# coganlab/cross_patient_speech_decoding

Hardware: AMD Instinct MI355X
Metric: ECoG trials/sec seq2seq-RNN training (higher is better)
Workload: dtype bf16x3; 1 GPU; configs[3] per-GPU shard: 8-patient MCCA-aligned input (d = 30), enc 2x bi-GRU H=512, dec 1x GRU, T=200 (T'=20), F=100, full-batch step of 2048 trials per GPU (8 patients x 2048 trials over 8 GPUs), dropout 0.3, teacher forcing 0.5, clip 0.5, AdamW; trials_per_gpu=2048, global_batch=2048, parallelism=dp1, collective=none (single process)

## Files before the change

cross_patient_speech_decoding_amd/nn_models/functional.py:

```python
import ctypes as C
from typing import NamedTuple

import torch

from .._dev import need_gpu as _need_gpu, ptr as _ptr, ptr_array as _ptr_array, stream as _stream, workspace as _ws
from .. import _switches
from .._lib import TnProblem, call, lib, rowmap

_f32 = torch.float32

GEMM_PRECISIONS = {'fp32': 0, 'bf16x3': 1}


def set_gemm_precision(name):
    if name not in GEMM_PRECISIONS:
        raise ValueError(f"gemm precision must be one of {sorted(GEMM_PRECISIONS)}")
    call('xps_set_gemm_precision', GEMM_PRECISIONS[name])


def get_gemm_precision():
    mode = lib().xps_get_gemm_precision()
    return {v: k for k, v in GEMM_PRECISIONS.items()}[mode]


# ... 340 lines not shown
        return dgi, dghn, dh0
    call('xps_gru_seq_bwd_f32', _ptr(dy), _ptr(dhn), _ptr(y_ext), _ptr(saved), _ptr_array(w_hh), _ptr_array(w_t), _ptr(dgi),
         _ptr(dghn), _ptr(dh0), T, B, H, ndir, _ptr(ws), nbytes, _stream())
    return dgi, dghn, dh0


def _recurrent_grad_problems(dgi, dghn, y_ext, w_hh_params, b_hh_params, T, B, H, ndir, fmt=0, y_fmt=0):
    dev = y_ext.device
    ldy = ndir * H
    probs, rets = [], []
    for d in range(ndir):
        dw, db, acc_w, rw, rb = _grad_targets(w_hh_params[d], (3 * H, H), b_hh_params[d], (3 * H,), dev)
        first_slot = 0 if d == 0 else 2
        hprev = y_ext.view(-1)[first_slot * B * ldy + d * H:]
        probs.append(tn_problem(dgi[d], hprev, dw, 2 * H, H, T * B, ra=rowmap(3 * H, fmt=fmt), rb=rowmap(ldy, fmt=y_fmt), rc=rowmap(H),
                                colsum_out=db, accumulate=acc_w))
        probs.append(tn_problem(dghn[d], hprev, dw[2 * H:], H, H, T * B, ra=rowmap(H, fmt=fmt), rb=rowmap(ldy, fmt=y_fmt), rc=rowmap(H),
                                colsum_out=db[2 * H:], accumulate=acc_w))
        rets.append((rw, rb))
    return probs, rets


class GRURecurFn(torch.autograd.Function):

    @staticmethod
    def forward(ctx, gi, h0, ndir, *wb):
        _need_gpu(gi, h0, *wb)
        w_hh = [w.contiguous() for w in wb[:ndir]]
        b_hh = [b.contiguous() for b in wb[ndir:]]
        gi = gi.contiguous()
        _, T, B, H3 = gi.shape
        H = H3 // 3
        h0c = None if h0 is None else h0.contiguous()
        save = any(ctx.needs_input_grad)
        y_ext, saved = _gru_forward(gi, w_hh, b_hh, h0c, T, B, H, ndir, save)
        if save:
            ctx.save_for_backward(y_ext, saved, *w_hh)
            ctx.form = saved.launch_form
        ctx.params = wb
        ctx.dims = (T, B, H, ndir)
        ctx.has_h0 = h0 is not None
        return y_ext

    @staticmethod
    def backward(ctx, dy_ext):
        y_ext, saved, *w_hh = ctx.saved_tensors
        T, B, H, ndir = ctx.dims
        need_dh0 = ctx.has_h0 and ctx.needs_input_grad[1]
        dgi, dghn, dh0 = _gru_backward(dy_ext[1:T + 1], None, y_ext, saved, w_hh, T, B, H, ndir, need_dh0, form=ctx.form)
        if need_dh0:
            dh0[0] += dy_ext[0, :, :H]
            if ndir == 2:
                dh0[1] += dy_ext[T + 1, :, H:]
        probs, rets = _recurrent_grad_problems(dgi, dghn, y_ext, ctx.params[:ndir], ctx.params[ndir:], T, B, H, ndir)
        gemm_tn_grouped(probs, y_ext.device)
        return (dgi, dh0, None, *[r[0] for r in rets], *[r[1] for r in rets])


HN_NONE, HN_STACK, HN_SUM = 0, 1, 2


FMT_X_SPLIT4, FMT_Y_SPLIT4 = 1, 2


def split4_mode():
    return lib().xps_get_gemm_precision() == 1 and bool(_switches.get('XPS_SPLIT4'))


def layer_output_split4_ok(T, B, H, ndir, drop_p):
    return bool(drop_p and drop_p > 0.0 and split4_mode() and H > 256 and (ndir * H) % 4 == 0
                and not fused_dropout_supported(T, B, H, ndir))


def _presplit_weights_ok(rows, In, H3):
    return (split4_mode() and In % 4 == 0 and rows >= 4096 and In * H3 >= _switches.get('XPS_SPLIT4_WEIGHTS_MIN')
            and bool(_switches.get('XPS_SPLIT4_WEIGHTS')))


def skinny_dx_wanted(rows, In, K):
    return (bool(_switches.get('XPS_SKINNY_DX')) and split4_mode() and In % 4 == 0 and In < 256 and rows % 256 == 0
            and rows >= 96 * 256 and K % 32 == 0 and K >= 512 and bool(_switches.get('XPS_GEMM_DMA')))


def split4_pad(w, ldo):
    w = w.contiguous()
    out = torch.empty(w.shape[0], ldo, dtype=_f32, device=w.device)
    call('xps_split4_pad_f32', _ptr(w), w.shape[1], w.shape[0], w.shape[1], _ptr(out), ldo, _stream())
    return out


def split4(x, drop_p=0.0, seed=0):
    out = torch.empty_like(x)
    call('xps_split4_f32', _ptr(x), _ptr(out), x.numel(), float(drop_p), int(seed), _stream())
    return out


class GruPlan(NamedTuple):
    cluster_on: bool
    precision: int
    drop_fused: bool
    x_fmt: int
    w_fmt: int
    y_out_split: bool
    fwd_images: bool
    fwd_ysplit: bool
    want_dropped: bool
    bwd_split4: int
    y_fmt: int
    skinny_dx: bool


def gru_layer_plan(T, B, In, H, ndir, drop_p, fmt):
    has_drop = bool(drop_p and drop_p > 0.0)
    drop_fused = bool(has_drop and fused_dropout_supported(T, B, H, ndir))
    y_out_split = bool(fmt & FMT_Y_SPLIT4)
    if y_out_split and (not has_drop or drop_fused):
        raise ValueError('FMT_Y_SPLIT4: only with a separate dropout pass (see layer_output_split4_ok)')
    w_fmt = 1 if _presplit_weights_ok(T * B, In, 3 * H) else 0
    split4 = bool(split4_wanted(T, B, H, ndir))
    hprev = bool(hprev_split_wanted(T, B, H, ndir, split4))
    fwd_images = bool(fwd_images_wanted(T, B, H, ndir, hprev))
    return GruPlan(cluster_on=lib().xps_get_gru_cluster_mode() != 0, precision=lib().xps_get_gemm_precision(), drop_fused=drop_fused,
                   x_fmt=1 if (fmt & FMT_X_SPLIT4) else 0, w_fmt=w_fmt, y_out_split=y_out_split, fwd_images=fwd_images,
                   fwd_ysplit=bool(fwd_ysplit_wanted(T, B, H, ndir, hprev)), want_dropped=fwd_images and y_out_split,
                   bwd_split4=int(split4), y_fmt=int(hprev),
                   skinny_dx=bool(split4 and not w_fmt and skinny_dx_wanted(T * B, In, 3 * H)))


class GRULayerFmtFn(torch.autograd.Function):

    @staticmethod
    def forward(ctx, x, ndir, hn_mode, drop_p, fmt, *wb):
        ctx.set_materialize_grads(False)
        _need_gpu(x, *wb)
        x = x.contiguous()
        T, B, In = x.shape
        w_ih = [wb[4 * d + 0].contiguous() for d in range(ndir)]
        w_hh = [wb[4 * d + 1].contiguous() for d in range(ndir)]
        b_ih = [wb[4 * d + 2].contiguous() for d in range(ndir)]
        b_hh = [wb[4 * d + 3].contiguous() for d in range(ndir)]
        H = w_hh[0].shape[1]
        plan = ctx.plan = gru_layer_plan(T, B, In, H, ndir, drop_p, fmt)
        gi = torch.empty(ndir, T, B, 3 * H, dtype=_f32, device=x.device)
        if plan.w_fmt:
            w_ih = [split4(w) for w in w_ih]
        ra, rb, rc = rowmap(In, fmt=plan.x_fmt), rowmap(In, fmt=plan.w_fmt), rowmap(3 * H)
        call('xps_gemm_nt_multi_f32', _ptr(x), C.byref(ra), _ptr_array(w_ih), C.byref(rb), _ptr_array([gi[d] for d in range(ndir)]),
             C.byref(rc), _ptr_array(b_ih), ndir, T * B, 3 * H, In, _stream())
        save = any(ctx.needs_input_grad)
        drop = None
        y_drop = None
        if drop_p and drop_p > 0.0:
            drop = (float(drop_p), next_dropout_seed())
        ctx.drop = drop
        y_split = None
        if (save and (plan.fwd_images or plan.fwd_ysplit)) or plan.want_dropped:
            y_ext, saved, y_split, y_drop = _gru_forward_images(gi, w_hh, b_hh, T, B, H, ndir, save, plan.want_dropped, drop)
        elif plan.drop_fused:
            y_ext, saved, y_drop = _gru_forward(gi, w_hh, b_hh, None, T, B, H, ndir, save, drop)
        else:
            y_ext, saved = _gru_forward(gi, w_hh, b_hh, None, T, B, H, ndir, save)
        if save:
            ctx.save_for_backward(x, y_ext, saved, *w_ih, *w_hh, *([y_split] if y_split is not None else []))
        ctx.params = wb
        ctx.dims = (T, B, H, ndir, In, hn_mode)
        y = y_ext[1:T + 1]
        if y_drop is not None:
            y = y_drop
        elif drop is not None:
            out = torch.empty(T, B, ndir * H, dtype=_f32, device=x.device)
            if plan.y_out_split:
                call('xps_split4_f32', _ptr(y), _ptr(out), out.numel(), drop[0], drop[1], _stream())
            else:
                call('xps_dropout_f32', _ptr(y), _ptr(out), None, out.numel(), drop[0], drop[1], _stream())
            y = out
        if hn_mode == HN_NONE:
            hn = None
        elif hn_mode == HN_SUM:
            hn = y_ext[T, :, :H] + y_ext[1, :, H:] if ndir == 2 else y_ext[T, :, :H].clone()
        else:
            hn = torch.stack([y_ext[T, :, :H]] + ([y_ext[1, :, H:]] if ndir == 2 else []), dim=0)
        return y, hn

    @staticmethod
    def backward(ctx, dy, dhn):
        T, B, H, ndir, In, hn_mode = ctx.dims
        if dhn is not None and hn_mode == HN_SUM:
            dhn = dhn.unsqueeze(0).expand(ndir, B, H).contiguous()
        plan = ctx.plan
        if lib().xps_get_gemm_precision() != plan.precision:
            names = {v: k for k, v in GEMM_PRECISIONS.items()}
            raise RuntimeError(f'GRU backward: the forward chose its operand formats in {names[plan.precision]} mode but the backward '
                               f'runs in {names[lib().xps_get_gemm_precision()]} mode: the product precision (set_gemm_precision / '
                               'XPS_GEMM_PRECISION) must not change between a forward and its backward')
        x, y_ext, saved, *w = ctx.saved_tensors
        y_split = w.pop() if (plan.fwd_images or plan.fwd_ysplit) else None
        w_ih, w_hh = w[:ndir], w[ndir:]
        fmt, y_fmt, x_fmt, w_fmt = plan.bwd_split4, plan.y_fmt, plan.x_fmt, plan.w_fmt
        wb = ctx.params
        if ctx.drop is not None and dy is not None and not plan.drop_fused:
            dyc = dy.contiguous()
            dyd = torch.empty_like(dyc)
            call('xps_dropout_f32', _ptr(dyc), _ptr(dyd), None, dyc.numel(), ctx.drop[0], ctx.drop[1], _stream())
            dy = dyd
        dgi, dghn, _ = _gru_backward(dy, dhn, y_ext, saved, w_hh, T, B, H, ndir, False, ctx.drop if plan.drop_fused else None,
                                     split4=bool(fmt), form=(plan.cluster_on, B, H))
        dev = x.device
        have_img = y_split is not None
        y_src = (y_split if have_img else torch.empty_like(y_ext)) if y_fmt else y_ext
        probs, rets_hh = _recurrent_grad_problems(dgi, dghn, y_src, [wb[4 * d + 1] for d in range(ndir)],
                                                  [wb[4 * d + 3] for d in range(ndir)], T, B, H, ndir, fmt, y_fmt)
        rets_ih = []
        for d in range(ndir):
            dw, db, acc_w, rw, rb = _grad_targets(wb[4 * d + 0], (3 * H, In), wb[4 * d + 2], (3 * H,), dev)
            probs.append(tn_problem(dgi[d], x, dw, 3 * H, In, T * B, ra=rowmap(3 * H, fmt=fmt), rb=rowmap(In, fmt=x_fmt),
                                    colsum_out=db, accumulate=acc_w))
            rets_ih.append((rw, rb))
        direct = all(r[0] is None and r[1] is None for r in rets_ih + rets_hh)
        def launch_group(st):
            if y_fmt and not have_img:
                call('xps_split4_f32', _ptr(y_ext), _ptr(y_src), y_ext.numel(), 0.0, 0, _stream() if st is None else st)
            return gemm_tn_grouped(probs, dev, st)
        _launch_weight_grads(launch_group, dev, (dgi, dghn, x, y_ext, y_src), direct)
        dx = None
        if ctx.needs_input_grad[0]:
            dx = torch.empty(T, B, In, dtype=_f32, device=dev)
            if plan.skinny_dx:
                w_ih = [split4_pad(w, 256) for w in w_ih]
                w_fmt, ldw = 1, 256
            else:
                ldw = In
            if ndir == 2:
                ra, rb, rc = rowmap(3 * H, fmt=fmt), rowmap(ldw, fmt=w_fmt), rowmap(In)
                call('xps_gemm_nn2_f32', _ptr(dgi[0]), _ptr(w_ih[0]), 3 * H, _ptr(dgi[1]), _ptr(w_ih[1]), 3 * H,
                     C.byref(ra), C.byref(rb), _ptr(dx), C.byref(rc), T * B, In, 0, _stream())
            else:
                gemm_nn(dgi[0], w_ih[0], dx, T * B, In, 3 * H, ra=rowmap(3 * H, fmt=fmt), rb=rowmap(ldw, fmt=w_fmt))
        grads = []
        for d in range(ndir):
            grads += [rets_ih[d][0], rets_hh[d][0], rets_ih[d][1], rets_hh[d][1]]
        return (dx, None, None, None, None, *grads)


class GRULayerDropFn(torch.autograd.Function):

    @staticmethod
    def forward(ctx, x, ndir, hn_mode, drop_p, *wb):
        return GRULayerFmtFn.forward(ctx, x, ndir, hn_mode, drop_p, 0, *wb)

    @staticmethod
    def backward(ctx, dy, dhn):
        g = GRULayerFmtFn.backward(ctx, dy, dhn)
        return g[:4] + g[5:]


class GRULayerFn(torch.autograd.Function):

    @staticmethod
    def forward(ctx, x, ndir, hn_mode, *wb):
        return GRULayerDropFn.forward(ctx, x, ndir, hn_mode, 0.0, *wb)

    @staticmethod
    def backward(ctx, dy, dhn):
        g = GRULayerDropFn.backward(ctx, dy, dhn)
        return g[:3] + g[4:]


POST_SYNCBN_HOOKS = []
def _dp_world(group):
    import torch.distributed as dist
    if group is not None and dist.is_available() and dist.is_initialized():
        return dist.get_world_size(group)
    return 1


def _dp_enabled(group):
    return _dp_world(group) > 1


def _dist_sum_(t, group):
    if _dp_enabled(group):
        import torch.distributed as dist
        dist.all_reduce(t, op=dist.ReduceOp.SUM, group=group)
        return True
    return False


def _global_rows(rows, group, device, global_trials, Tp):
    if global_trials is not None:
        return float(global_trials) * Tp
    cnt = torch.tensor([float(rows)], dtype=torch.float64, device=device)
    _dist_sum_(cnt, group)
    return float(cnt.item())


class TemporalConvFn(torch.autograd.Function):

    @staticmethod
    def forward(ctx, x, conv_w, conv_b, gamma, beta, running_mean, running_var, stride, training,
                relu, drop_mask, drop_scale, momentum, eps, group, global_trials=None, num_batches_tracked=None):
        _need_gpu(x, conv_w)
        x = x.contiguous()
        B, T, Cin = x.shape
        F, _, k = conv_w.shape
        Tp = (T - k) // stride + 1
        if Tp < 1:
            raise ValueError('TemporalConv: sequence shorter than the kernel')
        w2 = conv_w.permute(0, 2, 1).contiguous().view(F, k * Cin)
        rows = Tp * B
        y = torch.empty(Tp, B, F, dtype=_f32, device=x.device)
        ra = rowmap(stride * Cin, rpg=Tp, gs=T * Cin)
        rc = rowmap(B * F, rpg=Tp, gs=F)
        gemm_nt(x, w2, y, rows, F, k * Cin, bias=conv_b, ra=ra, rc=rc)
        out = torch.empty_like(y)
        if training:
            stats = torch.empty(2 * F, dtype=_f32, device=x.device)
            nbytes = lib().xps_colsum_f32_workspace(rows, F)
            ws = _ws(nbytes, x.device)
            call('xps_colsum_f32', _ptr(y), F, rows, F, _ptr(stats), None, 0, _ptr(ws), nbytes, _stream())
            count = float(rows)
# ... 729 lines not shown
```

include/xps.h:

```cpp
#ifndef XPS_H
#define XPS_H

#include <stddef.h>
#include <stdint.h>

#ifdef __cplusplus
extern "C" {
#endif

#define XPS_OK 0
#define XPS_E_INVALID (-1)
#define XPS_E_HIP (-2)
#define XPS_E_WORKSPACE (-3)

typedef struct xps_rowmap {
    int64_t gs;
    int64_t ld;
    int32_t rpg;
    int32_t fmt;
} xps_rowmap;
#define XPS_FMT_F32 0
#define XPS_FMT_SPLIT4 1

const char* xps_last_error(void);
int xps_abi_version(void);
int xps_stream_create_low_priority(void** stream);
int xps_stream_destroy(void* stream);
int xps_set_switch(const char* name, long long value);
int xps_get_switch(const char* name, long long* value);
int xps_list_switches(char* buf, size_t n);
int xps_set_gemm_precision(int mode);
int xps_get_gemm_precision(void);
int xps_set_gemm_big_tiles(int on);
int xps_get_gemm_big_tiles(void);


int xps_gemm_nt_f32(const float* A, const xps_rowmap* ra, const float* B, const xps_rowmap* rb,
                    float* C, const xps_rowmap* rc, const float* bias,
                    int M, int N, int K, int accumulate, void* stream);
int xps_gemm_nn_f32(const float* A, const xps_rowmap* ra, const float* B, const xps_rowmap* rb,
                    float* C, const xps_rowmap* rc,
                    int M, int N, int K, int accumulate, void* stream);
int xps_gemm_nt_multi_f32(const float* A, const xps_rowmap* ra, const float* const* B, const xps_rowmap* rb,
                          float* const* C, const xps_rowmap* rc, const float* const* bias, int nprob,
                          int M, int N, int K, void* stream);
int xps_gemm_nn2_f32(const float* A1, const float* B1, int K1, const float* A2, const float* B2, int K2,
                     const xps_rowmap* ra, const xps_rowmap* rb, float* C, const xps_rowmap* rc,
                     int M, int N, int accumulate, void* stream);
size_t xps_gemm_tn_f32_workspace(int M, int N, int K);
int xps_gemm_tn_f32(const float* A, const xps_rowmap* ra, const float* B, const xps_rowmap* rb,
                    float* C, const xps_rowmap* rc,
                    int M, int N, int K, int accumulate,
                    void* workspace, size_t workspace_bytes, void* stream);

typedef struct xps_tn_problem {
    const float* A; const float* B; float* C; float* colsum_a;
    xps_rowmap ra, rb, rc;
    int32_t M, N, K, accumulate;
} xps_tn_problem;
size_t xps_gemm_tn_grouped_f32_workspace(const xps_tn_problem* probs, int n);
int xps_gemm_tn_grouped_f32(const xps_tn_problem* probs, int n, void* workspace, size_t workspace_bytes,
                            void* stream);

#define XPS_GEMM_FORM_NT 0
#define XPS_GEMM_FORM_NN 1
#define XPS_GEMM_FORM_NN2 2
#define XPS_GEMM_FORM_NT_MULTI 3
#define XPS_GEMM_ROUTE_REFUSED 0
#define XPS_GEMM_ROUTE_NONE 1
#define XPS_GEMM_ROUTE_SMALL_M 2
#define XPS_GEMM_ROUTE_SKINNY 3
#define XPS_GEMM_ROUTE_BIG 8
#define XPS_GEMM_ROUTE_BIG_DEEP 12
#define XPS_GEMM_ROUTE_BIG_DMA 13
#define XPS_GEMM_ROUTE_TILE 16
#define XPS_GEMM_ROUTE_TILE_128 1
#define XPS_GEMM_ROUTE_TILE_EDGE 2
#define XPS_GEMM_ROUTE_TILE_BF 4
#define XPS_GEMM_ROUTE_TILE_PRE 8
#define XPS_GEMM_ROUTE_PROJ_WS 32
int xps_gemm_route(int form, const float* A, const xps_rowmap* ra, const void* B, const xps_rowmap* rb, const float* A2,
                   const float* B2, const xps_rowmap* rc, int M, int N, int K, int K2, int nprob, int* lead_rows,
                   int* tail_route);
#define XPS_GEMM_TN_CLASS_128 0
#define XPS_GEMM_TN_CLASS_BIG 1
#define XPS_GEMM_TN_CLASS_BIG_DMA 2
#define XPS_GEMM_ROUTE_TN_EDGE 1
#define XPS_GEMM_ROUTE_TN_BF 2
#define XPS_GEMM_ROUTE_TN_PRE 4
#define XPS_GEMM_ROUTE_TN_DEEP 8
#define XPS_GEMM_ROUTE_TN_UNIFORM 16
#define XPS_GEMM_ROUTE_TN_FLAT 32
int xps_gemm_tn_grouped_route(const xps_tn_problem* probs, int n, int* cls, int* splits, int* kchunk);

size_t xps_colsum_f32_workspace(int rows, int cols);
int xps_colsum_f32(const float* X, int64_t ldx, int rows, int cols, float* out, float* out_sq,
                   int accumulate, void* workspace, size_t workspace_bytes, void* stream);

size_t xps_gru_seq_fwd_f32_workspace(int T, int B, int H, int ndir);
long long xps_gru_seq_status_offset(int T, int B, int H, int ndir);
int xps_gru_set_status_word(unsigned* device_word);
int xps_set_gru_bptt_grid(int two_dimensional);
int xps_get_gru_bptt_grid(void);
int xps_set_gru_cluster_mode(int mode);
int xps_get_gru_cluster_mode(void);
int xps_gru_seq_fwd_f32(const float* gi, const float* const* w_hh, const float* const* b_hh,
                        const float* h0, float* y_ext, float* saved,
                        int T, int B, int H, int ndir, void* workspace, size_t workspace_bytes, void* stream);

size_t xps_gru_seq_bwd_f32_workspace(int T, int B, int H, int ndir);
int xps_gru_seq_bwd_f32(const float* dy, const float* dhn, const float* y_ext, const float* saved,
                        const float* const* w_hh, const float* const* w_hh_t, float* dgi, float* dghn, float* dh0,
                        int T, int B, int H, int ndir, void* workspace, size_t workspace_bytes, void* stream);
#define XPS_GRU_MAX_H_TILE 624
#define XPS_GRU_MAX_H_STEP 1264
#define XPS_GRU_ROUTE_REFUSED 0
#define XPS_GRU_ROUTE_CLUSTER 1
#define XPS_GRU_ROUTE_RESIDENT 2
#define XPS_GRU_ROUTE_GENERIC_VEC 3
#define XPS_GRU_ROUTE_GENERIC_SCALAR 4
#define XPS_GRU_ROUTE_STEP 8
#define XPS_GRU_ROUTE_STEP_VECA 1
#define XPS_GRU_ROUTE_STEP_VECB 2
int xps_gru_seq_route(int T, int B, int H, int ndir, int weights_aligned16, int backward);
int xps_gru_seq_fused_dropout_supported(int T, int B, int H, int ndir);
int xps_gru_seq_fwd_drop_f32(const float* gi, const float* const* w_hh, const float* const* b_hh,
                             const float* h0, float* y_ext, float* saved,
                             int T, int B, int H, int ndir, float* y_drop, float drop_p, uint64_t drop_seed,
                             void* workspace, size_t workspace_bytes, void* stream);
int xps_gru_seq_bwd_drop_f32(const float* dy, const float* dhn, const float* y_ext, const float* saved,
                             const float* const* w_hh, const float* const* w_hh_t, float* dgi, float* dghn, float* dh0,
                             int T, int B, int H, int ndir, float drop_p, uint64_t drop_seed,
                             void* workspace, size_t workspace_bytes, void* stream);
int xps_gru_seq_fwd_images_supported(int T, int B, int H, int ndir);
int xps_gru_seq_fwd_image_exchange_supported(int T, int B, int H, int ndir);
int xps_gru_seq_fwd_images_f32(const float* gi, const float* const* w_hh, const float* const* b_hh,
                               const float* h0, float* y_ext, float* saved, int T, int B, int H, int ndir,
                               float* y_split, float* y_drop_split, float drop_p, uint64_t drop_seed,
                               void* workspace, size_t workspace_bytes, void* stream);
int xps_gru_seq_bwd_split4_supported(int T, int B, int H, int ndir);
int xps_gru_seq_bwd_split4_f32(const float* dy, const float* dhn, const float* y_ext, const float* saved,
                               const float* const* w_hh, const float* const* w_hh_t, float* dgi, float* dghn, float* dh0,
                               int T, int B, int H, int ndir, float drop_p, uint64_t drop_seed,
                               void* workspace, size_t workspace_bytes, void* stream);

int xps_transpose_f32(const float* src, float* dst, int rows, int cols, void* stream);
int xps_transpose_batched_f32(const float* const* src, float* const* dst, int n, int rows, int cols, void* stream);

int xps_bn_centered_sumsq_f32(const float* y, int rows, int F, const float* stats, double count, float* out_sq,
                              void* workspace, size_t workspace_bytes, void* stream);
int xps_bn_finalize_f32(const float* stats, double count, float* mean, float* rstd,
                        float* running_mean, float* running_var, int64_t* num_batches_tracked,
                        float momentum, float eps, int F, void* stream);
int xps_bn_apply_f32(const float* y, const float* mean, const float* rstd,
                     const float* gamma, const float* beta, const float* drop_mask, float drop_scale,
                     float* out, int64_t rows, int F, int relu, void* stream);
int xps_bn_finalize_apply_f32(const float* y, const float* stats, double count, const float* gamma, const float* beta,
                              float* mean, float* rstd, float* running_mean, float* running_var,
                              int64_t* num_batches_tracked, float momentum, float eps, const float* drop_mask,
                              float drop_scale, float* out, int64_t rows, int F, int relu, void* stream);
int xps_bn_apply_eval_f32(const float* y, const float* running_mean, const float* running_var, float eps,
                          const float* gamma, const float* beta, float* out,
                          int64_t rows, int F, int relu, void* stream);
size_t xps_bn_bwd_workspace(int64_t rows, int F);
int xps_bn_bwd_reduce_f32(const float* dout, const float* out, const float* y, const float* mean,
                          const float* rstd, const float* drop_mask, float drop_scale, int relu,
                          float* sums, float* dbeta_acc, float* dgamma_acc, int64_t rows, int F,
                          void* workspace, size_t workspace_bytes, void* stream);
int xps_bn_bwd_apply_f32(const float* dout, const float* out, const float* y, const float* mean,
                         const float* rstd, const float* gamma, const float* drop_mask,
                         float drop_scale, int relu, const float* sums, double count,
                         float* dy, int64_t rows, int F, void* stream);

int xps_decoder_supported(int H, int C, int L);
int xps_decoder_fwd_f32(const float* table, const float* w_hh, const float* b_hh, const float* h0,
                        const float* w_fc, const float* b_fc, const int64_t* teacher, const int32_t* flags,
// ... 277 lines not shown
```

Measured before the change: 321,100 trials/s.

## Add dedicated skinny input-gradient kernels for narrow-input GRU layers

```diff
diff --git a/cross_patient_speech_decoding_amd/csrc/xps_gru_inputgrad.hip b/cross_patient_speech_decoding_amd/csrc/xps_gru_inputgrad.hip
--- /dev/null
+++ b/cross_patient_speech_decoding_amd/csrc/xps_gru_inputgrad.hip
@@ -0,0 +1,462 @@
+#include "xps_common.h"
+#include "xps_gemm_tile.h"
+#include "xps_gemm_dma.h"
+using namespace xps_tile;
+namespace {
+
+constexpr int IG_SLABS = 256;
+constexpr int IG_MAX_RG = 5;
+constexpr int IG_D = 4;
+constexpr int IG_B_IMG = 32 * 512;
+constexpr int ig_stage_bytes(int rg) { return rg * 32 * 128 + IG_B_IMG; }
+
+struct DxArgs {
+    const float* dgi[2];
+    const float* w[2];
+    float* dx;
+    int rows, In, H3, ndir;
+};
+
+inline int dx_row_groups(long long rows) {
+    long long rg = (rows + 32LL * IG_SLABS - 1) / (32LL * IG_SLABS);
+    return rg < 1 ? 1 : rg > IG_MAX_RG ? IG_MAX_RG : (int)rg;
+}
+
+template <int RG, bool PRE>
+__global__ __launch_bounds__(512, 2) void gru_dx_slab_kernel(const DxArgs a) {
+    extern __shared__ __attribute__((aligned(16))) unsigned char smem[];
+    constexpr int R = 32 * RG, A_IMG = R * 128, STAGE = A_IMG + IG_B_IMG;
+    constexpr int NP = RG + 4;
+    constexpr int NG = 2 * RG;
+    const int tid = threadIdx.x, lane = tid & 63;
+    const int wave8 = __builtin_amdgcn_readfirstlane(tid >> 6);
+    const bool loader = wave8 >= 4;
+    const int wave = wave8 & 3;
+    const int row0 = blockIdx.x * R;
+    const int nsd = a.H3 / 32, ns = nsd * a.ndir;
+    const unsigned lds0 = xps_big::dma_lds_base(smem);
+    unsigned va[RG];
+#pragma unroll
+    for (int i = 0; i < RG; ++i) {
+        const int lr = 8 * (wave + 4 * i) + (lane >> 3);
+        const int key = (lr >> 1) & 7;
+        int gr = row0 + lr;
+        gr = gr < a.rows ? gr : a.rows - 1;
+        va[i] = (unsigned)((long long)(gr - row0) * a.H3 * 4 + (((lane & 7) ^ key) << 4));
+    }
+    const int ng = a.In >> 2;
+    const int bgrp = (lane & 31) < ng ? (lane & 31) : ng - 1;
+    unsigned vb[4];
+#pragma unroll
+    for (int j = 0; j < 4; ++j) vb[j] = (unsigned)(((2 * (wave + 4 * j) + (lane >> 5)) * a.In + 4 * bgrp) * 4);
+    auto piece = [&](int s, int pc) {
+        const int ss = s < ns ? s : ns - 1;
+        const int d = ss >= nsd ? 1 : 0, kk = ss - d * nsd;
+        const unsigned st = lds0 + (unsigned)(s % IG_D) * STAGE;
+        if (pc < RG) {
+            const unsigned char* base = reinterpret_cast<const unsigned char*>((d ? a.dgi[1] : a.dgi[0]) + (long long)row0 * a.H3 + kk * 32);
+            xps_big::dma_piece(base, va[pc], st + (unsigned)(wave + 4 * pc) * 1024u);
+        } else {
+            const unsigned char* base = reinterpret_cast<const unsigned char*>((d ? a.w[1] : a.w[0]) + (long long)kk * 32 * a.In);
+            xps_big::dma_piece(base, vb[pc - RG], st + A_IMG + (unsigned)(wave + 4 * (pc - RG)) * 1024u);
+        }
+    };
+    const int r = lane & 31, h = lane >> 5, fkey = (r >> 1) & 7;
+    int fka[2][2];
+#pragma unroll
+    for (int t = 0; t < 2; ++t)
+#pragma unroll
+        for (int j = 0; j < 2; ++j) fka[t][j] = r * 128 + (((4 * t + 2 * h + j) ^ fkey) << 4);
+    const int fb = A_IMG + (8 * h) * 512 + (32 * wave + r) * 4;
+    auto frag_a = [&](const unsigned char* st, int g, bf16x8& fh, bf16x8& fl) {
+        const int t = g / RG, i = g % RG;
+        const unsigned char* p = st + i * (32 * 128);
+        if (PRE) {
+            const bf16x8 ga = *reinterpret_cast<const bf16x8*>(p + fka[t][0]);
+            const bf16x8 gb = *reinterpret_cast<const bf16x8*>(p + fka[t][1]);
+            fh = __builtin_shufflevector(ga, gb, 0, 1, 2, 3, 8, 9, 10, 11);
+            fl = __builtin_shufflevector(ga, gb, 4, 5, 6, 7, 12, 13, 14, 15);
+        } else {
+            const f32x4 ga = *reinterpret_cast<const f32x4*>(p + fka[t][0]);
+            const f32x4 gb = *reinterpret_cast<const f32x4*>(p + fka[t][1]);
+#pragma unroll
+            for (int j = 0; j < 4; ++j) {
+                __bf16 x, y;
+                bf_split(ga[j], x, y); fh[j] = x; fl[j] = y;
+                bf_split(gb[j], x, y); fh[4 + j] = x; fl[4 + j] = y;
+            }
+        }
+    };
+    auto frag_b = [&](const unsigned char* st, int t, bf16x8& fh, bf16x8& fl) {
+        float v[8];
+#pragma unroll
+        for (int j = 0; j < 8; ++j) v[j] = *reinterpret_cast<const float*>(st + fb + (16 * t + j) * 512);
+#pragma unroll
+        for (int j = 0; j < 8; ++j) { __bf16 x, y; bf_split(v[j], x, y); fh[j] = x; fl[j] = y; }
+    };
+    static_assert(IG_D == 4, "the counted wait below leaves the pieces of two stages in flight");
+    if (loader) {
+#pragma unroll
+        for (int s = 0; s < IG_D - 1; ++s)
+#pragma unroll
+            for (int pc = 0; pc < NP; ++pc) piece(s, pc);
+        for (int s = 0; s < ns; ++s) {
+            asm volatile("s_waitcnt vmcnt(%0)" ::"n"(2 * NP) : "memory");
+            __builtin_amdgcn_s_barrier();
+#pragma unroll
+            for (int pc = 0; pc < NP; ++pc) piece(s + IG_D - 1, pc);
+        }
+        asm volatile("s_waitcnt vmcnt(0)" ::: "memory");
+        return;
+    }
+    f32x16 acc[RG];
+#pragma unroll
+    for (int i = 0; i < RG; ++i)
+#pragma unroll
+        for (int q = 0; q < 16; ++q) acc[i][q] = 0.f;
+    const bool active = 32 * wave < a.In;
+    for (int s = 0; s < ns; ++s) {
+        __builtin_amdgcn_s_barrier();
+        if (!active) continue;
+        const unsigned char* st = smem + (s % IG_D) * STAGE;
+        bf16x8 bh[2], bl[2], ah[2], al[2];
+        frag_b(st, 0, bh[0], bl[0]);
+        frag_b(st, 1, bh[1], bl[1]);
+        frag_a(st, 0, ah[0], al[0]);
+#pragma unroll
+        for (int g = 0; g < NG; ++g) {
+            const int t = g / RG, i = g % RG;
+            if (g + 1 < NG) frag_a(st, g + 1, ah[(g + 1) & 1], al[(g + 1) & 1]);
+            acc[i] = __builtin_amdgcn_mfma_f32_32x32x16_bf16(al[g & 1], bh[t], acc[i], 0, 0, 0);
+            acc[i] = __builtin_amdgcn_mfma_f32_32x32x16_bf16(ah[g & 1], bl[t], acc[i], 0, 0, 0);
+            acc[i] = __builtin_amdgcn_mfma_f32_32x32x16_bf16(ah[g & 1], bh[t], acc[i], 0, 0, 0);
+        }
+    }
+    if (!active) return;
+    const int col = 32 * wave + r;
+    if (col >= a.In) return;
+#pragma unroll
+    for (int i = 0; i < RG; ++i)
+#pragma unroll
+        for (int q = 0; q < 16; ++q) {
+            const int row = row0 + 32 * i + (q & 3) + 8 * (q >> 2) + 4 * h;
+            if (row < a.rows) __builtin_nontemporal_store(acc[i][q], a.dx + (long long)row * a.In + col);
+        }
+}
+
+template <int RG, bool PRE>
+int dx_launch(const DxArgs& a, hipStream_t st) {
+    static bool prepared = false;
+    constexpr int bytes = IG_D * ig_stage_bytes(RG);
+    if (!prepared) {
+        if (hipFuncSetAttribute(reinterpret_cast<const void*>(gru_dx_slab_kernel<RG, PRE>), hipFuncAttributeMaxDynamicSharedMemorySize, bytes) != hipSuccess)
+            return -1;
+        prepared = true;
+    }
+    const int blocks = (int)(((long long)a.rows + 32 * RG - 1) / (32 * RG));
+    hipLaunchKernelGGL((gru_dx_slab_kernel<RG, PRE>), dim3(blocks), dim3(512), bytes, st, a);
+    return 0;
+}
+
+template <bool PRE>
+int dx_dispatch(int rg, const DxArgs& a, hipStream_t st) {
+    switch (rg) {
+        case 1: return dx_launch<1, PRE>(a, st);
+        case 2: return dx_launch<2, PRE>(a, st);
+        case 3: return dx_launch<3, PRE>(a, st);
+        case 4: return dx_launch<4, PRE>(a, st);
+        default: return dx_launch<5, PRE>(a, st);
+    }
+}
+
+constexpr int DW_D = 3;
+constexpr int DW_B_IMG = 16 * 512;
+constexpr int DW_TILE = xps_big::DMA_IMG + DW_B_IMG;
+constexpr int DW_STAGE = 2 * DW_TILE;
+constexpr int DW_LDS = DW_D * DW_STAGE;
+constexpr int DW_NP = 6;
+
+struct DwArgs {
+    const float* dgi[2];
+    const float* x;
+    float* dw[2];
+    float* db[2];
+    float* ws;
+    int rows, In, H3, ndir, slices, ranges, range_rows, accumulate;
+};
+
+struct DwPlan { int slices, ranges, range_rows; };
+inline DwPlan dw_plan(int rows, int H3, int ndir) {
+    DwPlan p;
+    p.slices = (H3 + 255) / 256;
+    const int nc = p.slices * ndir;
+    int rs = IG_SLABS / nc;
+    const int cap = (rows + 127) / 128;
+    rs = rs > cap ? cap : rs;
+    rs = rs < 1 ? 1 : rs;
+    p.range_rows = ((rows + rs - 1) / rs + 31) / 32 * 32;
+    p.ranges = (rows + p.range_rows - 1) / p.range_rows;
+    return p;
+}
+inline size_t dw_ws_floats(const DwPlan& p, int In, int H3, int ndir) { return (size_t)p.ranges * ndir * H3 * (In + 1); }
+
+template <bool PRE>
+__global__ __launch_bounds__(768, 3) void gru_dw_cols_kernel(const DwArgs a) {
+    typedef __attribute__((address_space(3))) bf16x4 lds_bf16x4;
+    extern __shared__ __attribute__((aligned(16))) unsigned char smem[];
+    const int tid = threadIdx.x, lane = tid & 63;
+    const int wave = __builtin_amdgcn_readfirstlane(tid >> 6);
+    const int nc = a.slices * a.ndir;
+    const int cs = blockIdx.x % nc, rg = blockIdx.x / nc;
+    const int d = cs / a.slices, c0 = (cs % a.slices) * 256;
+    const int kbeg = rg * a.range_rows;
+    const int kend = min(a.rows, kbeg + a.range_rows);
+    const int nks = (kend - kbeg + 31) / 32;
+    const int wm = (wave >> 2) * 128, wn = (wave & 3) * 32;
+    const unsigned lds0 = xps_big::dma_lds_base(smem);
+    const float* A = d ? a.dgi[1] : a.dgi[0];
+    const unsigned va = (c0 + 4 * lane < a.H3) ? (unsigned)(lane * 16) : 0u;
+    const int ng = a.In >> 2;
+    const int bgrp = (lane & 31) < ng ? (lane & 31) : ng - 1;
+    auto piece = [&](int s, int pc, int v) {
+        const int brow = 2 * v + (lane >> 5);
+        const unsigned ra0 = (unsigned)xps_big::dma_rowoff(2 * v), ra1 = (unsigned)xps_big::dma_rowoff(2 * v + 1);
+        const int ks = s < nks ? s : nks - 1;
+        const int t = pc / 3, j = pc % 3;
+        const int kt0 = kbeg + 32 * ks + 16 * t;
+        const int k0 = kt0 < a.rows ? kt0 : a.rows - 1;
+        const unsigned st = lds0 + (unsigned)(s % DW_D) * DW_STAGE + (unsigned)t * DW_TILE;
+        if (j < 2) {
+            int gr = k0 + 2 * v + j;
+            gr = gr < a.rows ? gr : a.rows - 1;
+            xps_big::dma_piece(reinterpret_cast<const unsigned char*>(A + (long long)gr * a.H3 + c0), va, st + (j ? ra1 : ra0));
+        } else {
+            const int last = a.rows - 1 - k0;
+            const int rr = brow < last ? brow : last;
+            const unsigned vb = (unsigned)((rr * a.In + 4 * bgrp) * 4);
+            xps_big::dma_piece(reinterpret_cast<const unsigned char*>(a.x + (long long)k0 * a.In), vb,
+                               st + xps_big::DMA_IMG + (unsigned)v * 1024u);
+        }
+    };
+    const int r = lane & 31, h = lane >> 5;
+    const int g = lane >> 4, q = (lane >> 2) & 3, pp = lane & 3;
+    const int fro = xps_big::dma_rowoff(8 * (g >> 1) + q) + ((g & 1) * 4 + pp) * 16;
+    const int fa = fro + (wm / 4) * 16;
+    int fa32[8];
+#pragma unroll
+    for (int j = 0; j < 8; ++j) fa32[j] = xps_big::dma_rowoff(8 * h + j) + (wm + r) * 4;
+    const int fb = xps_big::DMA_IMG + (8 * h) * 512 + (wn + r) * 4;
+    auto frag_a = [&](const unsigned char* st, int i, bf16x8& fh, bf16x8& fl) {
+        if (PRE) {
+            const unsigned char* p = st + fa + i * 128;
+            const bf16x4 h0 = __builtin_amdgcn_ds_read_tr16_b64_v4bf16((lds_bf16x4*)(p));
+            const bf16x4 h1 = __builtin_amdgcn_ds_read_tr16_b64_v4bf16((lds_bf16x4*)(p + xps_big::DMA_ROW4));
+            const bf16x4 l0 = __builtin_amdgcn_ds_read_tr16_b64_v4bf16((lds_bf16x4*)(p + 8));
+            const bf16x4 l1 = __builtin_amdgcn_ds_read_tr16_b64_v4bf16((lds_bf16x4*)(p + xps_big::DMA_ROW4 + 8));
+            fh = __builtin_shufflevector(h0, h1, 0, 1, 2, 3, 4, 5, 6, 7);
+            fl = __builtin_shufflevector(l0, l1, 0, 1, 2, 3, 4, 5, 6, 7);
+        } else {
+#pragma unroll
+            for (int j = 0; j < 8; ++j) {
+                __bf16 x, y;
+                bf_split(*reinterpret_cast<const float*>(st + fa32[j] + i * 128), x, y);
+                fh[j] = x; fl[j] = y;
+            }
+        }
+    };
+    static_assert(DW_D == 3 && DW_NP == 6, "the counted wait below leaves the pieces of one stage in flight");
+    if (wave >= 8) {
+        const int l = wave - 8;
+#pragma unroll
+        for (int s = 0; s < DW_D - 1; ++s)
+#pragma unroll
+            for (int pc = 0; pc < 2 * DW_NP; ++pc) piece(s, pc % DW_NP, l + 4 * (pc / DW_NP));
+        for (int s = 0; s < nks; ++s) {
+            asm volatile("s_waitcnt vmcnt(12)" ::: "memory");
+            __builtin_amdgcn_s_barrier();
+#pragma unroll
+            for (int pc = 0; pc < 2 * DW_NP; ++pc) piece(s + DW_D - 1, pc % DW_NP, l + 4 * (pc / DW_NP));
+        }
+        asm volatile("s_waitcnt vmcnt(0)" ::: "memory");
+        return;
+    }
+    f32x16 acc[4], cacc;
+#pragma unroll
+    for (int i = 0; i < 4; ++i)
+#pragma unroll
+        for (int e = 0; e < 16; ++e) acc[i][e] = 0.f;
+#pragma unroll
+    for (int e = 0; e < 16; ++e) cacc[e] = 0.f;
+    const int csel = wave & 3;
+    const bool active = wn < a.In;
+    for (int s = 0; s < nks; ++s) {
+        __builtin_amdgcn_s_barrier();
+        const unsigned char* st = smem + (s % DW_D) * DW_STAGE;
+        bf16x8 bh[2], bl[2], ones[2], ah[2], al[2];
+#pragma unroll
+        for (int t = 0; t < 2; ++t) {
+            const int nvalid = kend - (kbeg + 32 * s + 16 * t);
+            float v[8];
+#pragma unroll
+            for (int j = 0; j < 8; ++j) v[j] = *reinterpret_cast<const float*>(st + t * DW_TILE + fb + j * 512);
+#pragma unroll
+            for (int j = 0; j < 8; ++j) {
+                const bool ok = 8 * h + j < nvalid;
+                __bf16 x, y;
+                bf_split(ok ? v[j] : 0.f, x, y);
+                bh[t][j] = x; bl[t][j] = y;
+                ones[t][j] = (__bf16)(ok ? 1.0f : 0.0f);
+            }
+        }
+        frag_a(st, 0, ah[0], al[0]);
+#pragma unroll
+        for (int g = 0; g < 8; ++g) {
+            const int t = g >> 2, i = g & 3;
+            if (g + 1 < 8) frag_a(st + ((g + 1) >> 2) * DW_TILE, (g + 1) & 3, ah[(g + 1) & 1], al[(g + 1) & 1]);
+            if (active) {
+                acc[i] = __builtin_amdgcn_mfma_f32_32x32x16_bf16(al[g & 1], bh[t], acc[i], 0, 0, 0);
+                acc[i] = __builtin_amdgcn_mfma_f32_32x32x16_bf16(ah[g & 1], bl[t], acc[i], 0, 0, 0);
+                acc[i] = __builtin_amdgcn_mfma_f32_32x32x16_bf16(ah[g & 1], bh[t], acc[i], 0, 0, 0);
+            }
+            if (i == csel) {
+                cacc = __builtin_amdgcn_mfma_f32_32x32x16_bf16(al[g & 1], ones[t], cacc, 0, 0, 0);
+                cacc = __builtin_amdgcn_mfma_f32_32x32x16_bf16(ah[g & 1], ones[t], cacc, 0, 0, 0);
+            }
+        }
+    }
+    float* wslab = a.ws + ((size_t)(rg * a.ndir + d) * a.H3) * a.In;
+    float* bslab = a.ws + (size_t)a.ranges * a.ndir * a.H3 * a.In + (size_t)(rg * a.ndir + d) * a.H3;
+    const int n = wn + r;
+    if (n < a.In) {
+#pragma unroll
+        for (int i = 0; i < 4; ++i)
+#pragma unroll
+            for (int e = 0; e < 16; ++e) {
+                const int m = c0 + wm + 32 * i + (e & 3) + 8 * (e >> 2) + 4 * h;
+                if (m < a.H3) wslab[(size_t)m * a.In + n] = acc[i][e];
+            }
+    }
+    if (r == 0) {
+#pragma unroll
+        for (int e = 0; e < 16; ++e) {
+            const int m = c0 + wm + 32 * csel + (e & 3) + 8 * (e >> 2) + 4 * h;
+            if (m < a.H3) bslab[m] = cacc[e];
+        }
+    }
+}
+
+__global__ __launch_bounds__(256) void gru_dw_reduce_kernel(const DwArgs a) {
+    const long long w4 = (long long)a.ndir * a.H3 * a.In / 4, nb = a.db[0] ? (long long)a.ndir * a.H3 : 0;
+    const long long i = (long long)blockIdx.x * 256 + threadIdx.x;
+    const size_t wstride = (size_t)a.ndir * a.H3 * a.In, bstride = (size_t)a.ndir * a.H3;
+    if (i < w4) {
+        const long long per = (long long)a.H3 * a.In / 4;
+        const int d = (int)(i / per);
+        const long long o = (i % per) * 4;
+        const float* s = a.ws + (size_t)d * a.H3 * a.In + o;
+        f32x4 sum = *reinterpret_cast<const f32x4*>(s);
+        for (int rg = 1; rg < a.ranges; ++rg) sum += *reinterpret_cast<const f32x4*>(s + rg * wstride);
+        float* dst = (d ? a.dw[1] : a.dw[0]) + o;
+#pragma unroll
+        for (int e = 0; e < 4; ++e) dst[e] = (a.accumulate & 1) ? dst[e] + sum[e] : sum[e];
+    } else if (i < w4 + nb) {
+        const long long j = i - w4;
+        const int d = (int)(j / a.H3);
+        const int m = (int)(j % a.H3);
+        const float* s = a.ws + (size_t)a.ranges * wstride + j;
+        float sum = s[0];
+        for (int rg = 1; rg < a.ranges; ++rg) sum += s[rg * bstride];
+        float* dst = (d ? a.db[1] : a.db[0]) + m;
+        if (a.accumulate & 3) sum += *dst;
+        *dst = sum;
+    }
+}
+
+inline bool ig_aligned16(const void* p) { return (reinterpret_cast<uintptr_t>(p) & 15) == 0; }
+
+}
+
+extern "C" int xps_gru_inputgrad_supported(int rows, int In, int H3, int ndir) {
+    return rows >= 1 && In >= 4 && In <= 128 && In % 4 == 0 && H3 >= 32 && H3 % 32 == 0 && H3 <= 65536 && (ndir == 1 || ndir == 2);
+}
+
+extern "C" int xps_gru_inputgrad_dx_f32(const float* const* dgi, const float* const* w_ih, float* dx, int rows, int In, int H3, int ndir,
+                                        int dgi_fmt, void* stream) {
+    XPS_CHECK_ARG(dgi && w_ih && dx, "null argument");
+    XPS_CHECK_ARG(xps_gru_inputgrad_supported(rows, In, H3, ndir),
+                  "unsupported shape: rows >= 1, In a multiple of 4 in 4..128, 3H a multiple of 32 up to 65536, 1 or 2 directions");
+    XPS_CHECK_ARG(dgi_fmt == XPS_FMT_F32 || dgi_fmt == XPS_FMT_SPLIT4, "dgi_fmt: XPS_FMT_F32 or XPS_FMT_SPLIT4");
+    XPS_CHECK_ARG(xps_internal_gemm_mode() == 1, "bf16x3 product mode only (xps_set_gemm_precision)");
+    DxArgs a;
+    a.dgi[1] = a.w[1] = nullptr;
+    for (int d = 0; d < ndir; ++d) {
+        XPS_CHECK_ARG(dgi[d] && w_ih[d], "null direction pointer");
+        XPS_CHECK_ARG(ig_aligned16(dgi[d]) && ig_aligned16(w_ih[d]), "dgi and W_ih must be 16-byte aligned");
+        a.dgi[d] = dgi[d];
+        a.w[d] = w_ih[d];
+    }
+    a.dx = dx;
+    a.rows = rows; a.In = In; a.H3 = H3; a.ndir = ndir;
+    const int rg = dx_row_groups(rows);
+    const int lrc = dgi_fmt == XPS_FMT_SPLIT4 ? dx_dispatch<true>(rg, a, (hipStream_t)stream) : dx_dispatch<false>(rg, a, (hipStream_t)stream);
+    if (lrc) {
+        xps_set_error("xps_gru_inputgrad_dx_f32: cannot reserve %d bytes of LDS", IG_D * ig_stage_bytes(rg));
+        return XPS_E_HIP;
+    }
+    XPS_CHECK_LAUNCH();
+    return XPS_OK;
+}
+
+extern "C" size_t xps_gru_inputgrad_dw_workspace(int rows, int In, int H3, int ndir) {
+    if (!xps_gru_inputgrad_supported(rows, In, H3, ndir)) return 0;
+    return dw_ws_floats(dw_plan(rows, H3, ndir), In, H3, ndir) * sizeof(float);
+}
+
+extern "C" int xps_gru_inputgrad_dw_f32(const float* const* dgi, const float* x, float* const* dw, float* const* db, int rows, int In, int H3,
+                                        int ndir, int dgi_fmt, int x_fmt, int accumulate, void* workspace, size_t workspace_bytes,
+                                        void* stream) {
+    XPS_CHECK_ARG(dgi && x && dw && workspace, "null argument");
+    XPS_CHECK_ARG(xps_gru_inputgrad_supported(rows, In, H3, ndir),
+                  "unsupported shape: rows >= 1, In a multiple of 4 in 4..128, 3H a multiple of 32 up to 65536, 1 or 2 directions");
+    XPS_CHECK_ARG(dgi_fmt == XPS_FMT_F32 || dgi_fmt == XPS_FMT_SPLIT4, "dgi_fmt: XPS_FMT_F32 or XPS_FMT_SPLIT4");
+    XPS_CHECK_ARG(x_fmt == XPS_FMT_F32, "x must hold plain fp32 (XPS_FMT_F32)");
+    XPS_CHECK_ARG(accumulate >= 0 && accumulate <= 3, "accumulate: bit 0 = dW and db, bit 1 = db alone");
+    XPS_CHECK_ARG(xps_internal_gemm_mode() == 1, "bf16x3 product mode only (xps_set_gemm_precision)");
+    const DwPlan p = dw_plan(rows, H3, ndir);
+    if (workspace_bytes < dw_ws_floats(p, In, H3, ndir) * sizeof(float)) {
+        xps_set_error("xps_gru_inputgrad_dw_f32: workspace too small (%zu < %zu)", workspace_bytes, dw_ws_floats(p, In, H3, ndir) * sizeof(float));
+        return XPS_E_WORKSPACE;
+    }
+    XPS_CHECK_ARG(ig_aligned16(workspace) && ig_aligned16(x), "x and the workspace must be 16-byte aligned");
+    DwArgs a;
+    a.dgi[1] = nullptr; a.dw[1] = a.db[0] = a.db[1] = nullptr;
+    for (int d = 0; d < ndir; ++d) {
+        XPS_CHECK_ARG(dgi[d] && dw[d] && (!db || db[d]), "null direction pointer");
+        XPS_CHECK_ARG(ig_aligned16(dgi[d]), "dgi must be 16-byte aligned");
+        a.dgi[d] = dgi[d];
+        a.dw[d] = dw[d];
+        a.db[d] = db ? db[d] : nullptr;
+    }
+    a.x = x;
+    a.ws = static_cast<float*>(workspace);
+    a.rows = rows; a.In = In; a.H3 = H3; a.ndir = ndir;
+    a.slices = p.slices; a.ranges = p.ranges; a.range_rows = p.range_rows; a.accumulate = accumulate;
+    static bool prepared = false;
+    if (!prepared) {
+        if (hipFuncSetAttribute(reinterpret_cast<const void*>(gru_dw_cols_kernel<true>), hipFuncAttributeMaxDynamicSharedMemorySize, DW_LDS) != hipSuccess ||
+            hipFuncSetAttribute(reinterpret_cast<const void*>(gru_dw_cols_kernel<false>), hipFuncAttributeMaxDynamicSharedMemorySize, DW_LDS) != hipSuccess) {
+            xps_set_error("xps_gru_inputgrad_dw_f32: cannot reserve %d bytes of LDS", DW_LDS);
+            return XPS_E_HIP;
+        }
+        prepared = true;
+    }
+    hipStream_t st = (hipStream_t)stream;
+    const int blocks = p.slices * ndir * p.ranges;
+    if (dgi_fmt == XPS_FMT_SPLIT4) hipLaunchKernelGGL(gru_dw_cols_kernel<true>, dim3(blocks), dim3(768), DW_LDS, st, a);
+    else hipLaunchKernelGGL(gru_dw_cols_kernel<false>, dim3(blocks), dim3(768), DW_LDS, st, a);
+    XPS_CHECK_LAUNCH();
+    const long long items = (long long)ndir * H3 * In / 4 + (long long)ndir * H3;
+    hipLaunchKernelGGL(gru_dw_reduce_kernel, dim3((unsigned)((items + 255) / 256)), dim3(256), 0, st, a);
+    XPS_CHECK_LAUNCH();
+    return XPS_OK;
+}
diff --git a/cross_patient_speech_decoding_amd/nn_models/functional.py b/cross_patient_speech_decoding_amd/nn_models/functional.py
--- a/cross_patient_speech_decoding_amd/nn_models/functional.py
+++ b/cross_patient_speech_decoding_amd/nn_models/functional.py
@@ -446,6 +446,16 @@
             and rows >= 96 * 256 and K % 32 == 0 and K >= 512 and bool(_switches.get('XPS_GEMM_DMA')))
 
 
+def input_grads_wanted(rows, In, H3, ndir, precision=None, x_fmt=0):
+    precision = lib().xps_get_gemm_precision() if precision is None else precision
+    return bool(precision == 1 and not x_fmt and In % 4 == 0 and In <= 128 and rows >= 4096 and H3 % 256 == 0
+                and lib().xps_gru_inputgrad_supported(rows, In, H3, ndir))
+
+
+def _aligned16(t):
+    return t if t.data_ptr() % 16 == 0 else t.clone()
+
+
 def split4_pad(w, ldo):
     w = w.contiguous()
     out = torch.empty(w.shape[0], ldo, dtype=_f32, device=w.device)
@@ -472,6 +482,7 @@
     bwd_split4: int
     y_fmt: int
     skinny_dx: bool
+    input_grads: bool = False
 
 
 def gru_layer_plan(T, B, In, H, ndir, drop_p, fmt):
@@ -484,11 +495,13 @@
     split4 = bool(split4_wanted(T, B, H, ndir))
     hprev = bool(hprev_split_wanted(T, B, H, ndir, split4))
     fwd_images = bool(fwd_images_wanted(T, B, H, ndir, hprev))
-    return GruPlan(cluster_on=lib().xps_get_gru_cluster_mode() != 0, precision=lib().xps_get_gemm_precision(), drop_fused=drop_fused,
-                   x_fmt=1 if (fmt & FMT_X_SPLIT4) else 0, w_fmt=w_fmt, y_out_split=y_out_split, fwd_images=fwd_images,
+    precision, x_fmt = lib().xps_get_gemm_precision(), 1 if (fmt & FMT_X_SPLIT4) else 0
+    skinny_dx = bool(split4 and not w_fmt and skinny_dx_wanted(T * B, In, 3 * H))
+    return GruPlan(cluster_on=lib().xps_get_gru_cluster_mode() != 0, precision=precision, drop_fused=drop_fused,
+                   x_fmt=x_fmt, w_fmt=w_fmt, y_out_split=y_out_split, fwd_images=fwd_images,
                    fwd_ysplit=bool(fwd_ysplit_wanted(T, B, H, ndir, hprev)), want_dropped=fwd_images and y_out_split,
-                   bwd_split4=int(split4), y_fmt=int(hprev),
-                   skinny_dx=bool(split4 and not w_fmt and skinny_dx_wanted(T * B, In, 3 * H)))
+                   bwd_split4=int(split4), y_fmt=int(hprev), skinny_dx=skinny_dx,
+                   input_grads=not skinny_dx and input_grads_wanted(T * B, In, 3 * H, ndir, precision, x_fmt))
 
 
 class GRULayerFmtFn(torch.autograd.Function):
@@ -574,32 +587,55 @@
         y_src = (y_split if have_img else torch.empty_like(y_ext)) if y_fmt else y_ext
         probs, rets_hh = _recurrent_grad_problems(dgi, dghn, y_src, [wb[4 * d + 1] for d in range(ndir)],
                                                   [wb[4 * d + 3] for d in range(ndir)], T, B, H, ndir, fmt, y_fmt)
-        rets_ih = []
+        rets_ih, ih = [], []
         for d in range(ndir):
             dw, db, acc_w, rw, rb = _grad_targets(wb[4 * d + 0], (3 * H, In), wb[4 * d + 2], (3 * H,), dev)
-            probs.append(tn_problem(dgi[d], x, dw, 3 * H, In, T * B, ra=rowmap(3 * H, fmt=fmt), rb=rowmap(In, fmt=x_fmt),
-                                    colsum_out=db, accumulate=acc_w))
+            if plan.input_grads:
+                ih.append((dw, db, acc_w))
+            else:
+                probs.append(tn_problem(dgi[d], x, dw, 3 * H, In, T * B, ra=rowmap(3 * H, fmt=fmt), rb=rowmap(In, fmt=x_fmt),
+                                        colsum_out=db, accumulate=acc_w))
             rets_ih.append((rw, rb))
         direct = all(r[0] is None and r[1] is None for r in rets_ih + rets_hh)
+        x_al = _aligned16(x) if ih else x
         def launch_group(st):
             if y_fmt and not have_img:
                 call('xps_split4_f32', _ptr(y_ext), _ptr(y_src), y_ext.numel(), 0.0, 0, _stream() if st is None else st)
-            return gemm_tn_grouped(probs, dev, st)
-        _launch_weight_grads(launch_group, dev, (dgi, dghn, x, y_ext, y_src), direct)
+            keep = gemm_tn_grouped(probs, dev, st)
+            if ih:
+                same = all(t[2] == ih[0][2] for t in ih)
+                for ds in ([list(range(ndir))] if same else [[d] for d in range(ndir)]):
+                    nbytes = _memo(('ig_ws', T * B, In, 3 * H, len(ds)), lambda: lib().xps_gru_inputgrad_dw_workspace(T * B, In, 3 * H, len(ds)))
+                    ws = _ws(nbytes, dev)
+                    call('xps_gru_inputgrad_dw_f32', _ptr_array([dgi[d] for d in ds]), _ptr(x_al), _ptr_array([ih[d][0] for d in ds]),
+                         _ptr_array([ih[d][1] for d in ds]), T * B, In, 3 * H, len(ds), fmt, 0, int(ih[ds[0]][2]), _ptr(ws), nbytes,
+                         _stream() if st is None else st)
+                    keep.append(ws)
+            return keep
+        if not plan.input_grads:
+            _launch_weight_grads(launch_group, dev, (dgi, dghn, x, x_al, y_ext, y_src), direct)
         dx = None
         if ctx.needs_input_grad[0]:
             dx = torch.empty(T, B, In, dtype=_f32, device=dev)
-            if plan.skinny_dx:
+            if plan.input_grads:
+                w_plain = [_aligned16(w) for w in ([wb[4 * d + 0].contiguous() for d in range(ndir)] if w_fmt else w_ih)]
+                call('xps_gru_inputgrad_dx_f32', _ptr_array([dgi[d] for d in range(ndir)]), _ptr_array(w_plain), _ptr(dx), T * B, In, 3 * H,
+                     ndir, fmt, _stream())
+            elif plan.skinny_dx:
                 w_ih = [split4_pad(w, 256) for w in w_ih]
                 w_fmt, ldw = 1, 256
             else:
                 ldw = In
-            if ndir == 2:
+            if plan.input_grads:
+                pass
+            elif ndir == 2:
                 ra, rb, rc = rowmap(3 * H, fmt=fmt), rowmap(ldw, fmt=w_fmt), rowmap(In)
                 call('xps_gemm_nn2_f32', _ptr(dgi[0]), _ptr(w_ih[0]), 3 * H, _ptr(dgi[1]), _ptr(w_ih[1]), 3 * H,
                      C.byref(ra), C.byref(rb), _ptr(dx), C.byref(rc), T * B, In, 0, _stream())
             else:
                 gemm_nn(dgi[0], w_ih[0], dx, T * B, In, 3 * H, ra=rowmap(3 * H, fmt=fmt), rb=rowmap(ldw, fmt=w_fmt))
+        if plan.input_grads:
+            _launch_weight_grads(launch_group, dev, (dgi, dghn, x, x_al, y_ext, y_src), direct)
         grads = []
         for d in range(ndir):
             grads += [rets_ih[d][0], rets_hh[d][0], rets_ih[d][1], rets_hh[d][1]]
diff --git a/include/xps.h b/include/xps.h
--- a/include/xps.h
+++ b/include/xps.h
@@ -92,6 +92,13 @@
 #define XPS_GEMM_ROUTE_TN_UNIFORM 16
 #define XPS_GEMM_ROUTE_TN_FLAT 32
 int xps_gemm_tn_grouped_route(const xps_tn_problem* probs, int n, int* cls, int* splits, int* kchunk);
+
+int xps_gru_inputgrad_supported(int rows, int In, int H3, int ndir);
+int xps_gru_inputgrad_dx_f32(const float* const* dgi, const float* const* w_ih, float* dx, int rows, int In, int H3, int ndir,
+                             int dgi_fmt, void* stream);
+size_t xps_gru_inputgrad_dw_workspace(int rows, int In, int H3, int ndir);
+int xps_gru_inputgrad_dw_f32(const float* const* dgi, const float* x, float* const* dw, float* const* db, int rows, int In, int H3,
+                             int ndir, int dgi_fmt, int x_fmt, int accumulate, void* workspace, size_t workspace_bytes, void* stream);
 
 size_t xps_colsum_f32_workspace(int rows, int cols);
 int xps_colsum_f32(const float* X, int64_t ldx, int rows, int cols, float* out, float* out_sq,
```

New measurement: 317,800 trials/s. 1.0% lower.
